# vainglorygame/analyzer

Measured on AMD Instinct MI355X. Metric: matches/sec rated (whole node), 3v3 TrueSkill, 1M-player roster, higher is better.
Workload: dtype fp32; 1 GPU; global_batch=10000000, seq_len=6, players=1000000, matches_per_gpu=10000000, team_size=3, parallelism=dp1, mode=exact, bench_config=2, skew=1, force_merge=False

## Files before the change

### analyzer_amd/csrc/dataflow.hip

```cpp
#include <hip/hip_runtime.h>

#include "common.h"
#include "dataflow_dev.h"
#include "kernels.h"
#include "rate_core.h"
#include "rate_dev.h"
#include "telemetry_dev.h"

#ifndef ANA_HELD
#define ANA_HELD 1
#endif

namespace ana {

#ifndef ANA_LOCAL_HANDOFF
#define ANA_LOCAL_HANDOFF 1
#endif
constexpr bool kLocalHandoff = ANA_LOCAL_HANDOFF != 0;
#ifndef ANA_LOCAL_HANDOFF_MAXK
#define ANA_LOCAL_HANDOFF_MAXK 4
#endif


constexpr int kHeld = ANA_HELD;
#ifndef ANA_HELD5
#define ANA_HELD5 1
#endif
constexpr int kTeleInline = 64;

struct Batch {
  int32_t m = 0;
  int my_h = -1, my_bit = 0, mode = 0, n0 = 0, n1 = 0, rank0 = 1, rank1 = 1, first = 0, prevdup = -1;
  int32_t id = -1;
  bool inr = false, islast = false, own = false, any_dup = false;
  uint32_t lk0 = kNoMatch;
  v4i gs = {0, 0, 0, 0}, gm = {0, 0, 0, 0};
  int64_t toff = 0;
  int32_t tcnt = 0;
  bool tonly = false;
  uint8_t est = kRated;
};

template <int K, int G, int TELE, bool DIAG, int WPE = 1>
__global__ void __launch_bounds__(256) __attribute__((amdgpu_waves_per_eu(WPE)))
rate_dataflow_kernel(const int32_t* __restrict__ rec, const uint32_t* __restrict__ link,
                     int32_t* deps, float* state, const float* __restrict__ attrs,
                     float* __restrict__ first_prior, float* __restrict__ orows, int64_t orow,
                     uint32_t* ctrl,
                     RateParams prm, TelemetryParams tp) {
  constexpr int S = 2 * K;
  constexpr int R = S + 2;
  constexpr int kH = K >= 5 ? ANA_HELD5 : kHeld;
  constexpr bool kLH = kLocalHandoff && (K <= ANA_LOCAL_HANDOFF_MAXK || ANA_DIAG_BUILD != 0);
  constexpr bool TILES = TELE == 1;
  constexpr bool INL = TELE == 2;
  static_assert(G >= S && G <= 64, "a group holds one match");
  constexpr int NG = 64 / G;
  static_assert(kH >= 1 && kH <= 4, "held chunks");
  typedef uint32_t hvec __attribute__((ext_vector_type(kH <= 2 ? 2 : 4)));
  __shared__ hvec lloc[kWavesPerBlock][kLH ? kChunk : 1];
  constexpr int SPT = (4 + S + 3) / 4 * 4;
  constexpr int SP = SPT + (INL ? 4 : 0);
  constexpr int TT = INL ? ((kTeleInline + G - 1) / G < 8 ? (kTeleInline + G - 1) / G : 8) : 1;
  __shared__ __attribute__((aligned(16))) float tstat[kWavesPerBlock][INL ? NG : 1][INL ? S * kStatFeatures : 4];
  __shared__ __attribute__((aligned(16))) int32_t lpick[kWavesPerBlock][NG][SP];
  __shared__ float tele[kWavesPerBlock][TILES ? tele_scratch_floats<K>() : 1];
  constexpr int OQ = (5 * S + 2 + 3) / 4;
  __shared__ __attribute__((aligned(16))) float lrow[kWavesPerBlock][NG][4 * OQ];
  const int lane = threadIdx.x & 63;
  const int wv = threadIdx.x >> 6;
  const int j = lane % G;
  const int g = lane / G;
  const int gbase = lane - j;
  const uint64_t gmask = (((1ull << G) - 1ull) << gbase);
  const bool r0 = j < K;
  const int rpos = r0 ? j : j - K;
  const int64_t M = prm.num_matches;
  const int64_t P = prm.num_players;
  const float beta2 = prm.beta2, tau2 = prm.tau2, us = prm.unknown_sigma;
  const int epoch = prm.epoch_ptr ? __builtin_amdgcn_readfirstlane(*prm.epoch_ptr) : prm.epoch;
  const __amdgpu_buffer_rsrc_t rs =
      __builtin_amdgcn_make_buffer_rsrc(state, 0, (int)(P * kRowFloats * 4), 0x00020000);
  const __amdgpu_buffer_rsrc_t rl = __builtin_amdgcn_make_buffer_rsrc(
      const_cast<uint32_t*>(link), 0, (int)(M * S * 4), 0x00020000);
  const __amdgpu_buffer_rsrc_t rd = __builtin_amdgcn_make_buffer_rsrc(deps, 0, (int)(M * 4), 0x00020000);
  const int head = blockIdx.x % kHeads;
  uint64_t t0 = __builtin_amdgcn_s_memrealtime();
  uint32_t seen_progress = 0;
  const bool local_ok = kLH && prm.local_handoff != 0;
  uint32_t n_local = 0, n_global = 0, n_stale = 0;
  uint64_t d_issue = 0, d_wait = 0, d_after = 0, d_it0 = 0;
  uint64_t d_t[4] = {0, 0, 0, 0}, d_p[5] = {0, 0, 0, 0, 0};
  uint64_t d_s[4] = {0, 0, 0, 0}, d_i[3] = {0, 0, 0};
  uint32_t d_worked = 0, d_groups = 0, d_near = 0, d_pend = 0;

  int32_t hrec[kH][R];
  int64_t hoff[kH];
  int32_t hcnt[kH];
  int32_t cbase[kH];
  uint64_t pend[kH];
  uint32_t dval[kH];
  uint32_t need[kH];
#pragma unroll
  for (int h = 0; h < kH; ++h) {
    cbase[h] = -1;
    pend[h] = 0ull;
#pragma unroll
    for (int k = 0; k < R; ++k) hrec[h][k] = -1;
    dval[h] = kNone;
    need[h] = 0u;
    hoff[h] = 0;
    hcnt[h] = 0;
  }
  bool exhausted = false, tk_pending = false;
  unsigned tk = 0;
  uint32_t spins = 0, iter = 0;
  const bool tele_role = TILES && tp.role_stride > 0 && tp.impl != 0;
  const bool tele_inline = INL && tp.role_stride < 0 && tp.evoff != nullptr;
  const int tele_span = tele_role ? kTeleMaxSpan : kTeleTile;
  const int64_t tele_tiles = TILES && tp.evoff ? (tp.num_matches + tele_span - 1) / tele_span : 0;
  bool tele_done = tele_tiles == 0 || tele_inline;
  auto tele_claim = [&]() -> int64_t {
    unsigned t = 0;
    if (lane == 0)
      t = __hip_atomic_fetch_add((gu32*)&ctrl[12], 1u, __ATOMIC_RELAXED, __HIP_MEMORY_SCOPE_AGENT);
    t = __builtin_amdgcn_readfirstlane(t);
    return (int64_t)t < tele_tiles ? (int64_t)t : -1;
  };
  auto tele_run = [&](int64_t t) {
    if constexpr (TILES) {
      if (tele_role) telemetry_tile_mfma<K, 0, kTeleMaxSpan>(tp, t, lane, tele[wv], &ctrl[13]);
      else if (tp.impl) telemetry_tile_mfma<K>(tp, t, lane, tele[wv], &ctrl[13]);
      else telemetry_tile<K>(tp, t, lane, tele[wv], &ctrl[13]);
    }
  };
  if constexpr (TILES) {
    if (tele_role) {
      const int b = blockIdx.x, per = tp.role_stride >= 4 ? tp.role_stride / 4 : 1;
      const bool agg = tp.role_stride >= 4   ? (wv == ((b >> 3) & 3) && ((b >> 5) % per) == 0)
                       : tp.role_stride == 2 ? ((wv & 1) == ((b >> 3) & 1))
                                             : true;
      while (agg && !tele_done) {
        const int64_t t = tele_claim();
        if (t < 0) tele_done = true;
        else tele_run(t);
      }
    }
  }
  v2u tev_prev[TT];
#pragma unroll
  for (int t = 0; t < TT; ++t) tev_prev[t] = v2u{0u, 0u};
  int32_t tp_m = -1, tp_cnt = 0;
  int64_t tp_off = 0;
  auto tele_flush = [&]() {
    if constexpr (INL) {
      if (tp_m < 0) return;
      float* const ts = tstat[wv][g];
      typedef float v4f __attribute__((ext_vector_type(4)));
      if (j < S) {
        reinterpret_cast<v4f*>(ts)[2 * j] = v4f{0.f, 0.f, 0.f, 0.f};
        reinterpret_cast<v4f*>(ts)[2 * j + 1] = v4f{0.f, 0.f, 0.f, 0.f};
      }
      uint32_t nbad = 0;
      const uint32_t mtag = (uint32_t)tp_m & 0xffffu;
      auto fold = [&](v2u ev) {
        const int32_t meta = (int32_t)ev.x;
        const int slot = event_slot(meta);
        if (event_tag(meta) != mtag || slot >= S) {
          ++nbad;
          return;
        }
        float add;
        const int f = event_feature(event_type(meta), __uint_as_float(ev.y), add);
        if (f >= 0) atomicAdd(&ts[slot * kStatFeatures + f], add);
        atomicAdd(&ts[slot * kStatFeatures + kStatEvents], 1.f);
      };
#pragma unroll
      for (int t = 0; t < TT; ++t)
        if (j + G * t < tp_cnt) fold(tev_prev[t]);
      for (int e = j + G * TT; e < tp_cnt; e += G)
        fold(__builtin_nontemporal_load(reinterpret_cast<const v2u*>(tp.events + 2 * (tp_off + e))));
      if (j < S) {
        v4f* dst = reinterpret_cast<v4f*>(tp.stats + ((int64_t)tp_m * S + j) * kStatFeatures);
        __builtin_nontemporal_store(reinterpret_cast<const v4f*>(ts)[2 * j], dst);
        __builtin_nontemporal_store(reinterpret_cast<const v4f*>(ts)[2 * j + 1], dst + 1);
      }
      if (nbad) atomicAdd(&ctrl[13], nbad);
      tp_m = -1;
    }
  };
  const uint32_t max_spins = prm.idle_spins > 0 ? (uint32_t)prm.idle_spins : 0u;
  const int cl = prm.chunk_len;
  const int64_t nchunks = (M + cl - 1) / cl;

  for (;;) {
    if constexpr (DIAG) d_it0 = __builtin_amdgcn_s_memrealtime();
    uint64_t ready[kH];
    {
      hvec lv = {};
      if constexpr (kLH) lv = lloc[wv][lane];
#pragma unroll
      for (int h = 0; h < kH; ++h)
        ready[h] = __ballot(dval[h] != kNone && dval[h] + lv[h] == need[h]) & pend[h];
      if constexpr (DIAG) {
        uint32_t nn = 0, np = 0;
#pragma unroll
        for (int h = 0; h < kH; ++h) {
          nn += (uint32_t)__popcll(__ballot(dval[h] != kNone && dval[h] + lv[h] + 1u == need[h]) & pend[h]);
          np += (uint32_t)__popcll(pend[h]);
        }
        bool any = false;
#pragma unroll
        for (int h = 0; h < kH; ++h) any |= ready[h] != 0ull;
        if (any) {
          d_near += nn;
          d_pend += np;
        }
      }
    }
    __builtin_amdgcn_fence(__ATOMIC_ACQUIRE, "wavefront");
    if constexpr (DIAG) d_i[0] = __builtin_amdgcn_s_memrealtime();

    int my_h = -1, my_bit = 0, nassigned = 0;
#pragma unroll
    for (int h = 0; h < kH; ++h) {
      const uint64_t rdy = ready[h];
      if (rdy != 0ull && nassigned < NG) {
        const uint32_t below = __builtin_amdgcn_mbcnt_hi(
            (uint32_t)(rdy >> 32), __builtin_amdgcn_mbcnt_lo((uint32_t)rdy, 0u));
        const bool mine = ((rdy >> lane) & 1ull) && nassigned + (int)below < NG;
        if (mine) {
          int32_t w[SP];
          w[0] = cbase[h] + lane;
          w[1] = (h << 8) | lane;
          w[2] = hrec[h][S];
          w[3] = hrec[h][S + 1];
#pragma unroll
          for (int k = 0; k < SPT - 4; ++k) w[4 + k] = k < S ? hrec[h][k] : -1;
          if constexpr (INL) {
            w[SPT] = (int32_t)(uint32_t)hoff[h];
            w[SPT + 1] = (int32_t)(hoff[h] >> 32);
            w[SPT + 2] = hcnt[h];
            w[SPT + 3] = 0;
          }
          v4i* dst = reinterpret_cast<v4i*>(&lpick[wv][nassigned + (int)below][0]);
#pragma unroll
          for (int q = 0; q < SP / 4; ++q) dst[q] = v4i{w[4 * q], w[4 * q + 1], w[4 * q + 2], w[4 * q + 3]};
        }
        const uint64_t taken = __ballot(mine);
        pend[h] &= ~taken;
        nassigned += __popcll(taken);
      }
    }
    int32_t my_m = 0, my_id = -1;
    uint32_t my_m0 = 0u, my_m1 = 0u;
    int64_t my_toff = 0;
    int32_t my_tcnt = 0;
    if (g < nassigned) {
      const v4i pk = *reinterpret_cast<const v4i*>(&lpick[wv][g][0]);
      if constexpr (INL) {
        const v4i tk4 = *reinterpret_cast<const v4i*>(&lpick[wv][g][SPT]);
        my_toff = (int64_t)(((uint64_t)(uint32_t)tk4.y << 32) | (uint32_t)tk4.x);
        my_tcnt = tk4.z;
      }
      if (j < S) my_id = lpick[wv][g][4 + j];
      my_m = pk.x;
      my_h = (pk.y >> 8) & 255;
      my_bit = pk.y & 255;
      my_m0 = (uint32_t)pk.z;
      my_m1 = (uint32_t)pk.w;
    }
    const bool worked = nassigned > 0;
    if constexpr (DIAG) {
      d_worked += worked ? 1u : 0u;
      d_groups += (uint32_t)nassigned;
      d_i[1] = __builtin_amdgcn_s_memrealtime();
    }

    Batch nb;
    {
      const int32_t m = my_m;
      const uint32_t m0 = my_m0, m1 = my_m1;
      const int mode = meta_mode(m0);
      nb.my_h = my_h;
      nb.my_bit = my_bit;
      nb.m = m;
      nb.mode = mode;
      nb.n0 = meta_n0(m0);
      nb.n1 = meta_n1(m0);
      nb.rank0 = meta_winner0(m1) ? 0 : 1;
      nb.rank1 = meta_winner1(m1) ? 0 : 1;
      nb.tonly = INL && ((m1 >> 4) & 1u);
      nb.est = (uint8_t)(m1 >> 28);
      nb.tcnt = my_h >= 0 ? my_tcnt : 0;
      nb.toff = my_toff;
      const bool inr = my_h >= 0 && j < S && rpos < (r0 ? nb.n0 : nb.n1) && !nb.tonly;
      nb.inr = inr;
      const int32_t id = inr ? my_id : -1;
      nb.id = id;
      bool islast = true;
      int first = j, prevdup = -1;
      nb.any_dup = __ballot((m1 >> 3) & 1u) != 0ull;
      if (nb.any_dup) {
#pragma unroll
        for (int q = 0; q < S; ++q) {
          const int32_t oid = __shfl(id, gbase + q);
          if (id >= 0 && oid == id) {
            if (q < j) {
              if (first == j) first = q;
              prevdup = q;
            }
            if (q > j) islast = false;
          }
        }
      }
      nb.islast = islast;
      nb.first = first;
      nb.prevdup = prevdup;
      const bool own = inr && first == j;
      nb.own = own;
      const int goff = own ? id * (kRowFloats * 4) : kOutOfRange;
      nb.gs = __builtin_amdgcn_raw_buffer_load_b128(rs, goff, 0, 16);
      nb.gm = __builtin_amdgcn_raw_buffer_load_b128(rs, goff + 16 * (1 + mode), 0, 16);
      nb.lk0 = __builtin_amdgcn_raw_buffer_load_b32(rl, inr ? (m * S + j) * 4 : kOutOfRange, 0, 0);
    }

    if constexpr (DIAG) d_i[2] = __builtin_amdgcn_s_memrealtime();
    int staging = -1;
    int32_t r[R];
    uint32_t lks[S];
    int64_t stoff = 0;
    int32_t stcnt = 0;
#pragma unroll
    for (int k = 0; k < R; ++k) r[k] = -1;
#pragma unroll
    for (int k = 0; k < S; ++k) lks[k] = 0u;
    if (tk_pending) {
      const unsigned t = __builtin_amdgcn_readfirstlane(tk);
      tk_pending = false;
      const int64_t c = (int64_t)t * kHeads + head;
      if (prm.progress && lane == 0 &&
          ((c >= prm.progress_at && c < prm.progress_at + kHeads) ||
           (c >= nchunks && c < nchunks + kHeads)))
        __hip_atomic_store(prm.progress, prm.progress_value, __ATOMIC_RELAXED,
                           __HIP_MEMORY_SCOPE_SYSTEM);
      if (c * cl >= M) {
        exhausted = true;
      } else {
#pragma unroll
        for (int h = kH - 1; h >= 0; --h)
          if (cbase[h] < 0) staging = h;
#pragma unroll
        for (int h = 0; h < kH; ++h)
          if (h == staging) cbase[h] = (int32_t)(c * cl);
        const int64_t m = c * cl + lane;
        if (lane < cl && m < M) {
          const int32_t* src = rec + m * R;
          if constexpr (R % 4 == 0) {
#pragma unroll
            for (int k = 0; k < R / 4; ++k) {
              const v4i v = reinterpret_cast<const v4i*>(src)[k];
              r[4 * k] = v.x; r[4 * k + 1] = v.y; r[4 * k + 2] = v.z; r[4 * k + 3] = v.w;
            }
          } else {
#pragma unroll
            for (int k = 0; k < R; ++k) r[k] = src[k];
          }
          const v2u* ls = reinterpret_cast<const v2u*>(link + m * S);
#pragma unroll
          for (int k = 0; k < S / 2; ++k) {
            const v2u v = ls[k];
            lks[2 * k] = v.x;
            lks[2 * k + 1] = v.y;
          }
          if (tele_inline) {
            stoff = tp.evoff[m];
            stcnt = (int32_t)(tp.evoff[m + 1] - stoff);
          }
        }
      }
    }

    v2u tev_next[TT];
    int32_t tn_m = -1, tn_cnt = 0;
    int64_t tn_off = 0;
    auto notify = [&](uint32_t succ) {
      if (succ == kNoMatch) return;
      int lh = -1;
      int32_t lcb = 0;
      if (kLH && local_ok) {
#pragma unroll
        for (int h = 0; h < kH; ++h)
          if (cbase[h] >= 0 && (int32_t)succ >= cbase[h] && (int32_t)succ < cbase[h] + cl) {
            lh = h;
            lcb = cbase[h];
          }
      }
      if (kLH && lh >= 0) {
        atomicAdd(reinterpret_cast<uint32_t*>(&lloc[wv][(int32_t)succ - lcb]) + lh, 1u);
      } else {
        __hip_atomic_fetch_add((gu32*)(deps + succ), 1u, __ATOMIC_RELAXED, __HIP_MEMORY_SCOPE_AGENT);
      }
      const uint64_t lb = __ballot(lh >= 0);
      n_local += (uint32_t)__popcll(lb);
      n_global += (uint32_t)__popcll(__ballot(true) & ~lb);
    };
    auto rate_batch = [&](const Batch& bt) {
    int my_h = bt.my_h;
    const int my_bit = bt.my_bit;
    const int32_t m = bt.m;
    const int mode = bt.mode, n0 = bt.n0, n1 = bt.n1, rank0 = bt.rank0, rank1 = bt.rank1;
    const int first = bt.first, prevdup = bt.prevdup;
    const int32_t id = bt.id;
    const bool inr = bt.inr, islast = bt.islast, own = bt.own, any_dup = bt.any_dup;
    const uint32_t lk0 = bt.lk0;
    const v4i gs = bt.gs, gm = bt.gm;
    const uint32_t sa = (uint32_t)gs.y;
    const bool s_this = (sa & 0xffu) == (uint32_t)epoch;
    const uint32_t counters = s_this ? sa >> 8 : 0u;
    const uint32_t cnt = (counters >> (4 * mode)) & 15u;
    const bool shared_ok = !(lk0 & kLinkHasPred) || (s_this && (uint32_t)gs.w == (uint32_t)m);
    const bool mode_ok = cnt == 0u || (gm.y == epoch && (uint32_t)gm.w == cnt);
    const bool fresh = !own || (shared_ok && mode_ok);
    const bool overtaken =
        own && (((lk0 & kLinkHasPred) && s_this && (uint32_t)gs.w != kNoMatch &&
                 (uint32_t)gs.w > (uint32_t)m) ||
                (shared_ok && gm.y == epoch && (uint32_t)gm.w == (cnt == 15u ? 1u : cnt + 1u)));
    if (__ballot(overtaken) != 0ull && lane == 0) {
      atomicOr(&ctrl[2], 1u);
      atomicOr(&ctrl[18], 1u);
    }
    const uint64_t stale_lanes = __ballot(!fresh);
    if (stale_lanes) {
      const bool gstale = (stale_lanes & gmask) != 0ull;
      n_stale += (uint32_t)__popcll(__ballot(gstale && j == 0));
#pragma unroll
      for (int h = 0; h < kH; ++h) {
        uint64_t back = 0ull;
        for (int q = 0; q < NG; ++q) {
          const int bq = __shfl(gstale && my_h == h ? my_bit : -1, q * G);
          if (bq >= 0) back |= 1ull << bq;
        }
        pend[h] |= uniform64(back);
      }
      if (gstale) my_h = -1;
    }
    if constexpr (INL) {
      if (tele_inline && my_h >= 0) {
        tn_m = m;
        tn_cnt = bt.tcnt;
        tn_off = bt.toff;
      }
#pragma unroll
      for (int t = 0; t < TT; ++t) {
        const bool okl = tele_inline && my_h >= 0 && j + G * t < bt.tcnt;
        const int32_t* src = okl ? tp.events + 2 * (bt.toff + j + G * t)
                                 : reinterpret_cast<const int32_t*>(tp.evoff);
        tev_next[t] = __builtin_nontemporal_load(reinterpret_cast<const v2u*>(src));
      }
    }
    if (my_h >= 0) {
      const float smu = __int_as_float(gs.x), ssg = __int_as_float(gs.z);
      const float mmu = __int_as_float(gm.x), msg = __int_as_float(gm.z);
      const bool sh_null = smu != smu, md_null = mmu != mmu;
      float pms = smu, pss = ssg;
      bool seed_ok = true;
      if (__ballot(own && sh_null) != 0ull && own && sh_null) {
        const float4 at4 = reinterpret_cast<const float4*>(attrs)[id];
        const float attr[4] = {at4.x, at4.y, at4.z, at4.w};
        seed_ok = seed_prior<float>(attr, us, prm.vst, pms, pss);
      }
      const bool sh_bad = !sh_null && !(ssg == ssg && ssg != 0.f);
      const bool md_bad = !md_null && !(msg == msg && msg != 0.f);
      float pmm = md_null ? pms : mmu, psm = md_null ? pss : msg;
      uint32_t pflags = own ? ((sh_null ? 2u : 1u) | (md_null ? 4u : 0u)) : 0u;
      const uint8_t lst = !own ? (uint8_t)kRated
                               : (sh_null && !seed_ok) ? (uint8_t)kErrSeed
                               : (sh_bad || md_bad) ? (uint8_t)kErrSigma : (uint8_t)kRated;
      const uint64_t eb = __ballot(lst != kRated) & gmask;
      uint8_t gst = kRated;
      if (eb) gst = (uint8_t)__shfl((int)lst, (int)__builtin_ctzll(eb));
      float rsmu = smu, rssg = ssg, rmmu = mmu, rmsg = msg;
      uint32_t rcnt = counters;
      if (any_dup) {
        const int src = gbase + first;
        pms = __shfl(pms, src);
        pss = __shfl(pss, src);
        pmm = __shfl(pmm, src);
        psm = __shfl(psm, src);
        pflags = (uint32_t)__shfl((int)pflags, src);
        rsmu = __shfl(smu, src);
        rssg = __shfl(ssg, src);
        rcnt = (uint32_t)__shfl((int)counters, src);
        rmmu = __shfl(mmu, src);
        rmsg = __shfl(msg, src);
      }
      if (bt.tonly) gst = bt.est;
      if (gst == kRated && (n0 == 0 || n1 == 0)) gst = kErrEmptyRoster;
      float nsm = NAN, nss = NAN, nmm = NAN, nms = NAN, dl = NAN, q = NAN;
      if (gst == kRated) {
        if constexpr (DIAG) d_p[1] = __builtin_amdgcn_s_memrealtime();
        const float lsg = (r0 == (rank0 <= rank1)) ? 1.f : -1.f;
        f2 nm2, ns2;
        rate_pair<G>(f2{pms, pmm}, f2{pss, psm}, inr, lsg, n0 + n1, rank0 == rank1, beta2, tau2, j,
                     gbase, nm2, ns2, q);
        nsm = nm2.x;
        nmm = nm2.y;
        nss = ns2.x;
        nms = ns2.y;
        const bool bad_num = inr && !(isfinite(nsm) && isfinite(nss) && isfinite(nmm) &&
                                      isfinite(nms) && isfinite(q));
        if ((__ballot(bad_num) & gmask) != 0ull) gst = kErrNumeric;
        const float cur = nsm - nss;
        const float prevw = any_dup ? __shfl(cur, gbase + (prevdup >= 0 ? prevdup : j)) : cur;
        if (prevdup >= 0) dl = cur - prevw;
        else if (pflags & 1u) dl = cur - (pms - pss);
        else dl = 0.f;
      }
      const bool ok = gst == kRated && inr;
      if constexpr (DIAG) d_p[2] = __builtin_amdgcn_s_memrealtime();
      if (inr && islast) {
        const int off = id * (kRowFloats * 4);
        const uint32_t succ = lk0 & kMatchMask;
        const uint32_t c4 = (rcnt >> (4 * mode)) & 15u;
        const uint32_t c = c4 == 15u ? 1u : c4 + 1u;
        const uint32_t ncnt = (rcnt & ~(15u << (4 * mode))) | (c << (4 * mode));
        const uint32_t stag = (uint32_t)epoch | (ncnt << 8);
        __builtin_amdgcn_raw_buffer_store_b128(
            ok ? granule(nmm, (uint32_t)epoch, nms, c) : granule(rmmu, (uint32_t)epoch, rmsg, c),
            rs, off + 16 * (1 + mode), 0, 16);
        __builtin_amdgcn_raw_buffer_store_b128(
            ok ? granule(nsm, stag, nss, succ) : granule(rsmu, stag, rssg, succ),
            rs, off, 0, 16);
        notify(lk0 & kMatchMask);
      }
      if constexpr (DIAG) d_p[3] = __builtin_amdgcn_s_memrealtime();
      if (ok && prm.record_first_prior && own) {
        float* fp = first_prior + (int64_t)id * kRowFloats;
        if (pflags & 2u) { fp[0] = pms; fp[2] = pss; }
        if (pflags & 4u) { fp[4 * (1 + mode)] = pmm; fp[4 * (1 + mode) + 2] = psm; }
      }
      float* const orm = orows + (int64_t)m * orow;
      float* const lr = lrow[wv][g];
      if (j < S) {
        lr[j] = ok ? nsm : NAN;
        lr[S + j] = ok ? nss : NAN;
        lr[2 * S + j] = ok ? dl : NAN;
        lr[3 * S + j] = ok ? nmm : NAN;
        lr[4 * S + j] = ok ? nms : NAN;
      }
      if (j == 0) {
        lr[5 * S] = gst == kRated ? q : (gst == kAfk || gst == kInvalidRosters) ? 0.f : NAN;
        lr[5 * S + 1] = __uint_as_float((uint32_t)gst);
      }
      if (j == (G > 1 ? 1 : 0)) {
#pragma unroll
        for (int k = 5 * S + 2; k < 4 * OQ; ++k) lr[k] = 0.f;
      }
#pragma unroll
      for (int t = 0; t < (OQ + G - 1) / G; ++t) {
        typedef float v4f __attribute__((ext_vector_type(4)));
        const int qd = j + t * G;
        if (qd < OQ)
          __builtin_nontemporal_store(reinterpret_cast<const v4f*>(lr)[qd], reinterpret_cast<v4f*>(orm) + qd);
      }
    }
    };

    {
      bool free_slot = false;
#pragma unroll
      for (int h = 0; h < kH; ++h) free_slot |= cbase[h] < 0;
      if (free_slot && !exhausted) {
        if (lane == 0)
          tk = __hip_atomic_fetch_add((gu32*)&ctrl[4 + head], 1u, __ATOMIC_RELAXED,
                                      __HIP_MEMORY_SCOPE_AGENT);
        tk_pending = true;
      }
    }

    uint64_t d_w0 = 0, d_w1 = 0;
    if constexpr (DIAG) d_w0 = __builtin_amdgcn_s_memrealtime();
    asm volatile("s_waitcnt vmcnt(0)" ::: "memory");
    if constexpr (DIAG) d_w1 = __builtin_amdgcn_s_memrealtime();
    if constexpr (INL) {
#pragma unroll
      for (int t = 0; t < TT; ++t) asm volatile("" : "+v"(tev_prev[t]));
    }

    int64_t early_m = -1;
    uint8_t early_est = kRated;
    if (staging >= 0) {
      int64_t cb = 0;
#pragma unroll
      for (int h = 0; h < kH; ++h) if (h == staging) cb = cbase[h];
      const int64_t mm = lane < cl ? cb + lane : M;
      uint32_t nd = 0u;
      {
        const uint32_t m0s = (uint32_t)r[S];
        bool dup = false;
#pragma unroll
        for (int a = 0; a < S; ++a) {
          const bool ina = (a < K ? a : a - K) < (a < K ? meta_n0(m0s) : meta_n1(m0s));
          bool firsto = ina;
#pragma unroll
          for (int b = 0; b < a; ++b) {
            const bool inb = (b < K ? b : b - K) < (b < K ? meta_n0(m0s) : meta_n1(m0s));
            dup |= r[a] >= 0 && r[a] == r[b];
            if (inb && r[b] == r[a]) firsto = false;
          }
          if (firsto && (lks[a] & kLinkHasPred)) ++nd;
        }
        r[S + 1] = dup ? (r[S + 1] | 8) : (r[S + 1] & ~8);
      }
      const uint8_t est = mm < M ? early_status<K>(r, P) : kRated;
      const bool tonly = tele_inline && mm < M && est != kRated;
      if (tonly) r[S + 1] = (int32_t)(((uint32_t)r[S + 1] & 0x0fffffffu) | 16u | ((uint32_t)est << 28));
#pragma unroll
      for (int h = 0; h < kH; ++h)
        if (h == staging) {
#pragma unroll
          for (int k = 0; k < R; ++k) hrec[h][k] = r[k];
          hoff[h] = stoff;
          hcnt[h] = stcnt;
        }
      if constexpr (kLH) reinterpret_cast<uint32_t*>(&lloc[wv][lane])[staging] = 0u;
      if (mm < M && est != kRated && !tonly) {
        early_m = mm;
        early_est = est;
      }
      const uint64_t pm = __ballot(mm < M && (est == kRated || tonly));
#pragma unroll
      for (int h = 0; h < kH; ++h)
        if (h == staging) {
          pend[h] = pm;
          dval[h] = kNone;
          need[h] = tonly ? 0u : nd;
          if (pm == 0ull) cbase[h] = -1;
        }
    }

    if constexpr (DIAG) d_p[0] = d_p[1] = d_p[2] = d_p[3] = d_w1;
    rate_batch(nb);
    if (early_m >= 0) {
      typedef float v4f __attribute__((ext_vector_type(4)));
      const float qv = (early_est == kAfk || early_est == kInvalidRosters) ? 0.f : NAN;
      v4f* dst = reinterpret_cast<v4f*>(orows + early_m * orow);
#pragma unroll
      for (int q = 0; q < OQ; ++q) {
        float v[4];
#pragma unroll
        for (int i = 0; i < 4; ++i) {
          const int pos = 4 * q + i;
          v[i] = pos < 5 * S ? NAN : pos == 5 * S ? qv : pos == 5 * S + 1 ? __uint_as_float((uint32_t)early_est) : 0.f;
        }
        __builtin_nontemporal_store(v4f{v[0], v[1], v[2], v[3]}, dst + q);
      }
    }
    if constexpr (INL) {
      tele_flush();
#pragma unroll
      for (int t = 0; t < TT; ++t) tev_prev[t] = tev_next[t];
      tp_m = tn_m;
      tp_cnt = tn_cnt;
      tp_off = tn_off;
    }
    if constexpr (DIAG) {
      if (worked) {
        const uint64_t end = __builtin_amdgcn_s_memrealtime();
        d_issue += d_w0 - d_it0;
        d_wait += d_w1 - d_w0;
        d_after += end - d_w1;
        d_s[0] += d_i[0] - d_it0;
        d_s[1] += d_i[1] - d_i[0];
        d_s[2] += d_i[2] - d_i[1];
        d_s[3] += d_w0 - d_i[2];
        const uint64_t p1 = __builtin_amdgcn_readfirstlane((uint32_t)d_p[1]) |
                            ((uint64_t)__builtin_amdgcn_readfirstlane((uint32_t)(d_p[1] >> 32)) << 32);
        const uint64_t p2 = __builtin_amdgcn_readfirstlane((uint32_t)d_p[2]) |
                            ((uint64_t)__builtin_amdgcn_readfirstlane((uint32_t)(d_p[2] >> 32)) << 32);
        const uint64_t p3 = __builtin_amdgcn_readfirstlane((uint32_t)d_p[3]) |
                            ((uint64_t)__builtin_amdgcn_readfirstlane((uint32_t)(d_p[3] >> 32)) << 32);
        if (p1 >= d_w1 && p2 >= p1 && p3 >= p2 && end >= p3) {
          d_t[0] += p1 - d_w1;
          d_t[1] += p2 - p1;
          d_t[2] += p3 - p2;
          d_t[3] += end - p3;
        }
      }
    }

    ++iter;
#pragma unroll
    for (int h = 0; h < kH; ++h)
      dval[h] = __builtin_amdgcn_raw_buffer_load_b32(rd, ((pend[h] >> lane) & 1ull) ? (cbase[h] + lane) * 4 : kOutOfRange,
                                                     0, 16);

    {
      uint32_t retired = 0;
#pragma unroll
      for (int h = 0; h < kH; ++h)
        if (cbase[h] >= 0 && pend[h] == 0ull) {
          cbase[h] = -1;
          ++retired;
        }
      retired = __builtin_amdgcn_readfirstlane(retired);
      if (retired && lane == 0)
        __hip_atomic_fetch_add((gu32*)&ctrl[3], retired, __ATOMIC_RELAXED, __HIP_MEMORY_SCOPE_AGENT);
    }

    bool held = false;
#pragma unroll
    for (int h = 0; h < kH; ++h) held |= cbase[h] >= 0;
    if (exhausted && !held && !tk_pending) {
      tele_flush();
      if (lane == 0) {
        __hip_atomic_fetch_add((gu32*)&ctrl[15], iter, __ATOMIC_RELAXED, __HIP_MEMORY_SCOPE_AGENT);
        __hip_atomic_fetch_add((gu32*)&ctrl[26], n_local, __ATOMIC_RELAXED, __HIP_MEMORY_SCOPE_AGENT);
        __hip_atomic_fetch_add((gu32*)&ctrl[27], n_global, __ATOMIC_RELAXED, __HIP_MEMORY_SCOPE_AGENT);
        if (n_stale) __hip_atomic_fetch_add((gu32*)&ctrl[14], n_stale, __ATOMIC_RELAXED, __HIP_MEMORY_SCOPE_AGENT);
        if constexpr (DIAG) {
          __hip_atomic_fetch_add((gu32*)&ctrl[20], d_worked, __ATOMIC_RELAXED, __HIP_MEMORY_SCOPE_AGENT);
          __hip_atomic_fetch_add((gu32*)&ctrl[21], d_groups, __ATOMIC_RELAXED, __HIP_MEMORY_SCOPE_AGENT);
          __hip_atomic_fetch_add((gu32*)&ctrl[30], d_near, __ATOMIC_RELAXED, __HIP_MEMORY_SCOPE_AGENT);
          __hip_atomic_fetch_add((gu32*)&ctrl[31], d_pend, __ATOMIC_RELAXED, __HIP_MEMORY_SCOPE_AGENT);
          atomicAdd(reinterpret_cast<unsigned long long*>(&ctrl[22]), (unsigned long long)d_issue);
          atomicAdd(reinterpret_cast<unsigned long long*>(&ctrl[24]), (unsigned long long)d_wait);
          atomicAdd(reinterpret_cast<unsigned long long*>(&ctrl[28]), (unsigned long long)d_after);
          for (int q = 0; q < 4; ++q)
            atomicAdd(reinterpret_cast<unsigned long long*>(&ctrl[32 + 2 * q]), (unsigned long long)d_t[q]);
          for (int q = 0; q < 4; ++q)
            atomicAdd(reinterpret_cast<unsigned long long*>(&ctrl[40 + 2 * q]), (unsigned long long)d_s[q]);
        }
      }
      if constexpr (TILES) {
        while (!tele_done) {
          const int64_t t = tele_claim();
          if (t < 0) tele_done = true;
          else tele_run(t);
        }
      }
      break;
    }

    if (worked || staging >= 0) {
      spins = 0;
    } else {
      const uint64_t now = __builtin_amdgcn_s_memrealtime();
      if (now - t0 > kProgressTicks) {
        const uint32_t p = __hip_atomic_load((gu32*)&ctrl[3], __ATOMIC_RELAXED, __HIP_MEMORY_SCOPE_AGENT);
        if (p != seen_progress) {
          seen_progress = p;
          t0 = now;
        }
      }
      if (now - t0 > kTimeoutTicks) {
        if (lane == 0) {
          atomicOr(&ctrl[1], 1u);
          atomicOr(&ctrl[17], 1u);
        }
#pragma unroll
        for (int h = 0; h < kH; ++h)
          if (cbase[h] >= 0 && ((pend[h] >> lane) & 1ull))
            reinterpret_cast<uint8_t*>(orows + (int64_t)(cbase[h] + lane) * orow + 5 * S + 1)[0] = kNotProcessed;
        return;
      }
      if constexpr (TILES) {
        if (!tele_done && ((!tp.fused_tail && !tele_role) || !held)) {
          const int64_t t = tele_claim();
          if (t >= 0) {
            tele_run(t);
            spins = 0;
            continue;
          }
          tele_done = true;
        }
      }
      spins = spins < max_spins ? spins + 1u : max_spins;
      for (uint32_t k = 0; k < spins; ++k) __builtin_amdgcn_s_sleep(2);
    }
  }
}


__global__ void __launch_bounds__(64) zero_ctrl2_kernel(uint32_t* __restrict__ a, int na,
                                                        uint32_t* __restrict__ b, int nb) {
  if ((int)threadIdx.x < na) a[threadIdx.x] = 0u;
  if ((int)threadIdx.x < nb) b[threadIdx.x] = 0u;
}

int launch_rate(int K, const int32_t* rec, const uint32_t* link, int32_t* deps, float* state,
                const float* attrs, float* first_prior, const RateOut& out, uint32_t* ctrl,
                const RateParams& prm, const TelemetryParams& tp, int blocks, hipStream_t s) {
  const int64_t M = prm.num_matches;
  hipLaunchKernelGGL(zero_ctrl2_kernel, dim3(1), dim3(64), 0, s, ctrl + 1, prm.ctrl_ready ? 0 : 15,
                     ctrl + 20, 32);
  if (M <= 0) return 0;
  if (prm.chunk_len < 1 || prm.chunk_len > kChunk) return (int)hipErrorInvalidValue;
  if ((int64_t)prm.num_players * kRowFloats * 4 > kOutOfRange) return (int)hipErrorInvalidValue;
  if (M * 2 * K * 4 > kOutOfRange) return (int)hipErrorInvalidValue;
  if (!prm.epoch_ptr && (prm.epoch < 1 || prm.epoch > 255)) return (int)hipErrorInvalidValue;
  const int S = 2 * K;
  if (!(out.s_sig == out.s_mu + S && out.delta == out.s_mu + 2 * S && out.m_mu == out.s_mu + 3 * S &&
        out.m_sig == out.s_mu + 4 * S && out.quality == out.s_mu + 5 * S && out.qrow == out.row &&
        (void*)out.status == (void*)(out.s_mu + 5 * S + 1) && out.srow == out.row * 4))
    return (int)hipErrorInvalidValue;
  if (blocks < kHeads) blocks = kHeads;
  const bool tight = prm.tight_groups > 0 || (prm.tight_groups < 0 && K == 5);
#define ANA_RATE_LAUNCH_W(k, g, tele, diag, w)                                                     \
  hipLaunchKernelGGL((rate_dataflow_kernel<k, g, tele, diag, w>), dim3((unsigned)blocks), dim3(256), 0, s, \
                     rec, link, deps, state, attrs, first_prior, out.s_mu, out.row, ctrl, prm, tp)
#define ANA_RATE_LAUNCH_D(k, g, tele, diag)                                                        \
  do {                                                                                             \
    if constexpr (tele == 0 && !diag && k <= 3 && (g & (g - 1)) == 0) {                            \
      if (blocks > 256) ANA_RATE_LAUNCH_W(k, g, tele, diag, 4);           \
      else ANA_RATE_LAUNCH_W(k, g, tele, diag, 1);                                                 \
    } else {                                                                                       \
      ANA_RATE_LAUNCH_W(k, g, tele, diag, 1);                                                      \
    }                                                                                              \
  } while (0)
#define ANA_RATE_LAUNCH(k, g)                                      \
  do {                                                             \
    if (tp.evoff && tp.role_stride < 0) ANA_RATE_LAUNCH_D(k, g, 2, false); \
    else if (tp.evoff) ANA_RATE_LAUNCH_D(k, g, 1, false);          \
    else if (prm.diag) ANA_RATE_LAUNCH_D(k, g, 0, true);           \
    else ANA_RATE_LAUNCH_D(k, g, 0, false);                        \
  } while (0)
  switch (K) {
    case 1: ANA_RATE_LAUNCH(1, 2); break;
    case 2: ANA_RATE_LAUNCH(2, 4); break;
    case 3:
      if (tight) ANA_RATE_LAUNCH(3, 6);
      else ANA_RATE_LAUNCH(3, 8);
      break;
    case 4: ANA_RATE_LAUNCH(4, 8); break;
    case 5:
      if (tight) ANA_RATE_LAUNCH(5, 10);
      else ANA_RATE_LAUNCH(5, 16);
      break;
    default: return (int)hipErrorInvalidValue;
  }
#undef ANA_RATE_LAUNCH
#undef ANA_RATE_LAUNCH_D
  return (int)hipGetLastError();
}

}
```

### analyzer_amd/ops/rate.py

```python
from __future__ import annotations

import os
from dataclasses import dataclass
from typing import Dict, NamedTuple, Optional, Tuple

import torch

from ..config import MODES, N_TRACKS, EngineConfig, RaterConfig
from ..models.tiers import vst_table
from .native import native

RATED, AFK, INVALID_ROSTERS, UNSUPPORTED_MODE = 0, 1, 2, 3
ERR_SEED, ERR_SIGMA, ERR_EMPTY_ROSTER, ERR_NUMERIC, ERR_BAD_RECORD = 4, 5, 6, 7, 8
NOT_PROCESSED = 255
CTRL_WORDS = 52
STATUS_NAMES = {RATED: "rated", AFK: "afk", INVALID_ROSTERS: "invalid_rosters",
                UNSUPPORTED_MODE: "unsupported_mode", ERR_SEED: "error_seed",
                ERR_SIGMA: "error_sigma", ERR_EMPTY_ROSTER: "error_empty_roster",
                ERR_NUMERIC: "error_numeric", ERR_BAD_RECORD: "error_bad_record",
                NOT_PROCESSED: "not_processed"}
ERROR_STATUSES = (ERR_SEED, ERR_SIGMA, ERR_EMPTY_ROSTER, ERR_NUMERIC, ERR_BAD_RECORD)


class NativeRateError(RuntimeError):
    pass


class Schedule(NamedTuple):
    link: torch.Tensor
    deps: torch.Tensor

    NO_MATCH = 0x0FFFFFFF
    MATCH_MASK = 0x0FFFFFFF
    HAS_PRED = 1 << 30


@dataclass
class Roster:

    state: torch.Tensor
    attrs: torch.Tensor
    epoch: Optional[int] = None

    ROW = 32

    @property
    def num_players(self) -> int:
        return int(self.state.shape[0])

    @property
    def device(self) -> torch.device:
        return self.state.device

    @staticmethod
    def empty(num_players: int, device="cpu") -> "Roster":
        state = torch.zeros((num_players, 32), dtype=torch.float32, device=device)
        state[:, 0::2] = float("nan")
        attrs = torch.full((num_players, 4), float("nan"), dtype=torch.float32, device=device)
        attrs[:, 3] = 0.0
        return Roster(state, attrs, epoch=0)

    def tracks(self) -> torch.Tensor:
        return self.state.view(-1, 8, 4)[:, :, 0::2]

    def mu(self) -> torch.Tensor:
        return self.state[:, 0::4]

    def sigma(self) -> torch.Tensor:
        return self.state[:, 2::4]

    def track(self, name: str) -> torch.Tensor:
        idx = 0 if name in ("shared", "trueskill") else 1 + MODES.index(name.replace("trueskill_", ""))
        return self.state[:, 4 * idx:4 * idx + 3:2]

    def to(self, device) -> "Roster":
        return Roster(self.state.to(device), self.attrs.to(device), self.epoch)

    def clone(self) -> "Roster":
        return Roster(self.state.clone(), self.attrs.clone(), self.epoch)

    def next_epoch(self) -> int:
        if self.epoch is None or self.epoch >= 255:
            native().reset_tags(self.state)
            self.epoch = 0
        self.epoch += 1
        return self.epoch


@dataclass
class RateResult:

    quality: torch.Tensor
    status: torch.Tensor
    s_mu: torch.Tensor
    s_sig: torch.Tensor
    delta: torch.Tensor
    m_mu: torch.Tensor
    m_sig: torch.Tensor
    packed: Optional[torch.Tensor] = None

    FIELDS = ("quality", "status", "s_mu", "s_sig", "delta", "m_mu", "m_sig")

    @staticmethod
    def row_floats(K: int) -> int:
        return -(-(5 * 2 * K + 2) // 32) * 32

    @staticmethod
    def allocate(M: int, K: int, device, packed: bool = True) -> "RateResult":
        S = 2 * K
        if not packed:
            f = dict(dtype=torch.float32, device=device)
            return RateResult(torch.empty(M, **f), torch.empty(M, dtype=torch.uint8, device=device),
                              *(torch.empty((M, S), **f) for _ in range(5)))
        W = RateResult.row_floats(K)
        return RateResult.from_packed(torch.empty((M, W), dtype=torch.float32, device=device), K)

    @staticmethod
    def from_packed(buf: torch.Tensor, K: int) -> "RateResult":
        S = 2 * K
        if buf.dim() != 2 or buf.shape[1] != RateResult.row_floats(K) or buf.dtype != torch.float32 \
                or not buf.is_contiguous():
            raise ValueError("packed rows must be a contiguous fp32 [M, %d]" % RateResult.row_floats(K))
        slots = [buf[:, f * S:(f + 1) * S] for f in range(5)]
        status = buf.view(torch.uint8)[:, 4 * (5 * S + 1)]
        return RateResult(buf[:, 5 * S], status, *slots, packed=buf)

    @property
    def any_afk(self) -> torch.Tensor:
        return (self.status == AFK) | (self.status == INVALID_ROSTERS)

    def status_counts(self) -> Dict[str, int]:
        vals, counts = torch.unique(self.status.cpu(), return_counts=True)
        return {STATUS_NAMES.get(int(v), str(int(v))): int(c) for v, c in zip(vals, counts)}


class BatchRater:

    def __init__(self, cfg: Optional[RaterConfig] = None, host_fp64: bool = True,
                 blocks: Optional[int] = None):
        self.cfg = cfg or RaterConfig.from_env()
        self.host_fp64 = host_fp64
        ecfg = EngineConfig.from_env()
        self.fixed_blocks = int(blocks or ecfg.rate_blocks or 0)
        self.blocks = self.fixed_blocks or 512
        self.knobs = ecfg.rate_knobs()
        self.tele_fuse_max = int(ecfg.tele_fuse_max)
        self.chunk_cap = int(os.environ.get("ANA_RATE_CHUNK") or 0)
        self._vst: Dict[str, torch.Tensor] = {}
        self._ws: Dict[Tuple[str, str], torch.Tensor] = {}

    @staticmethod
    def has_telemetry(telemetry) -> bool:
        return telemetry is not None and telemetry[0].numel() > 0

    def tiles(self, telemetry, M: int) -> bool:
        return self.has_telemetry(telemetry) and self.knobs[5] >= 0

    def fuses(self, telemetry, M: int) -> bool:
        return self.has_telemetry(telemetry) and (self.knobs[5] >= 0 or M <= self.tele_fuse_max)

    def launch_blocks(self, K: int = 3, roster_bytes: int = 0) -> int:
        if self.fixed_blocks:
            return self.fixed_blocks
        return 256 if roster_bytes <= (256 << 20) else 512

    def chunk_len(self, M: int, telemetry: bool = False, blocks: Optional[int] = None, K: int = 3) -> int:
        if telemetry:
            return 64
        cap = self.chunk_cap if self.chunk_cap > 0 else (32 if K >= 5 else 64)
        need = -(-M // (4 * (blocks or self.blocks)))
        cl = 8
        while cl < need and cl < 64:
            cl *= 2
        return max(8, min(cl, cap))

    def grid_blocks(self, M: int, telemetry: bool = False, blocks: Optional[int] = None, K: int = 3) -> int:
        if telemetry:
            return self.blocks
        b = blocks or self.blocks
        chunks = -(-M // self.chunk_len(M, blocks=b, K=K))
        return max(1, min(b, -(-chunks // 4)))

    def vst(self, device) -> torch.Tensor:
        key = str(device)
        if key not in self._vst:
            self._vst[key] = torch.tensor(vst_table(), dtype=torch.float32, device=device)
        return self._vst[key]

    def _buffer(self, device, name: str, numel: int, dtype) -> torch.Tensor:
        key = (str(device), name)
        buf = self._ws.get(key)
        if buf is None or buf.numel() < numel or buf.dtype != dtype:
            buf = torch.empty(int(numel), dtype=dtype, device=device)
            self._ws[key] = buf
        return buf[:numel]

    def _ctrl(self, device) -> torch.Tensor:
        key = (str(device), "ctrl")
        buf = self._ws.get(key)
        if buf is None:
            buf = torch.zeros(CTRL_WORDS, dtype=torch.int32, device=device)
            self._ws[key] = buf
        return buf

    def schedule(self, rec: torch.Tensor, K: int, num_players: int,
                 tag: str = "", zero_ctrl: bool = False,
                 epoch_bump: Optional[torch.Tensor] = None, sort_nt: int = -1) -> Schedule:
        M = rec.shape[0]
        dev = rec.device
        link = self._buffer(dev, "link" + tag, M * 2 * K, torch.int32).view(M, 2 * K)
        deps = self._buffer(dev, "deps" + tag, M, torch.int32)
        if rec.is_cuda:
            nbytes = native().schedule_workspace_bytes(M * 2 * K, num_players)
            ws = self._buffer(dev, "sched_ws", nbytes, torch.uint8)
            ctrl = self._ctrl(dev)
        else:
            ws = torch.empty(0, dtype=torch.uint8)
            ctrl = torch.empty(0, dtype=torch.int32)
        bump = epoch_bump.data_ptr() if epoch_bump is not None and rec.is_cuda else 0
        native().schedule(rec, K, num_players, link, deps, ws, ctrl, bool(zero_ctrl and rec.is_cuda),
                          bump, int(sort_nt))
        return Schedule(link, deps)

    def rate(self, roster: Roster, rec: torch.Tensor, K: Optional[int] = None,
             out: Optional[RateResult] = None, first_prior: Optional[torch.Tensor] = None,
             check: bool = True, schedule: Optional[Schedule] = None,
             telemetry=None, progress=None, epoch_dev: Optional[torch.Tensor] = None) -> RateResult:
        K = int(K or (rec.shape[1] - 2) // 2)
        M = int(rec.shape[0])
        dev = rec.device
        if roster.device != dev:
            raise ValueError("roster is on %s but the stream is on %s" % (roster.device, dev))
        if out is None:
            out = RateResult.allocate(M, K, dev)
        P = roster.num_players
        cfg = self.cfg
        record = first_prior is not None
        fp = first_prior if record else torch.empty(0, dtype=torch.float32, device=dev)
        if dev.type == "cuda":
            ctrl_ready = schedule is None
            if schedule is None:
                schedule = self.schedule(rec, K, P, zero_ctrl=True, epoch_bump=epoch_dev)
            elif epoch_dev is not None:
                native().epoch_bump(epoch_dev)
            link, deps = schedule
            ctrl = self._ctrl(dev)
            epoch = roster.next_epoch() if epoch_dev is None else 1
        else:
            link = deps = ctrl = torch.empty(0, dtype=torch.int32)
            epoch = 1
            ctrl_ready = False
        blocks = self.launch_blocks(K, roster.state.numel() * roster.state.element_size())
        tiles = self.tiles(telemetry, M)
        after = None
        if self.has_telemetry(telemetry) and not self.fuses(telemetry, M) and dev.type == "cuda":
            after, telemetry = telemetry, None
        tele = self.has_telemetry(telemetry)
        if not tele:
            none = torch.empty(0, dtype=torch.int64, device=dev)
            telemetry = (none, none.to(torch.int32), none.to(torch.float32))
        native().rate(rec, K, link, deps, roster.state, roster.attrs, fp, out.quality, out.status,
                      out.s_mu, out.s_sig, out.delta, out.m_mu, out.m_sig, ctrl, self.vst(dev),
                      float(cfg.beta) ** 2, float(cfg.tau) ** 2, float(cfg.unknown_player_sigma),
                      record, self.grid_blocks(M, tiles, blocks, K), epoch,
                      self.host_fp64, *telemetry,
                      *(progress if progress is not None and dev.type == "cuda" else (0, 0, 0)),
                      epoch_dev.data_ptr() if epoch_dev is not None and dev.type == "cuda" else 0,
                      self.chunk_len(M, tiles, blocks, K), ctrl_ready, self.knobs)
        if after is not None:
            evoff, events, stats = after
            native().telemetry(evoff, events, K, stats, ctrl[13:14])
        if check and dev.type == "cuda":
            self.check_errors(dev)
        return out

    def stale_retries(self, device) -> int:
        return int(self._ctrl(device)[14].item())

    def iterations(self, device) -> int:
        return int(self._ctrl(device)[15].item())

    def handoffs(self, device) -> Tuple[int, int]:
        c = self._ctrl(device)[26:28].cpu()
        return int(c[0]), int(c[1])

    def diag(self, device) -> Dict[str, float]:
        c = [int(x) & 0xffffffff for x in self._ctrl(device).cpu().tolist()]
        u64 = lambda i: c[i] | (c[i + 1] << 32)
        worked = c[20]
        per = (lambda t: t * 0.01 / worked) if worked else (lambda t: 0.0)
        return {"wave_iterations": c[15], "worked_iterations": worked, "groups_assigned": c[21],
                "matches_per_worked_iteration": c[21] / worked if worked else 0.0,
                "issue_us": per(u64(22)), "wait_us": per(u64(24)), "after_us": per(u64(28)),
                "after_prior_us": per(u64(32)), "after_update_us": per(u64(34)),
                "after_publish_us": per(u64(36)), "after_rest_us": per(u64(38)),
                "issue_ready_us": per(u64(40)), "issue_assign_us": per(u64(42)),
                "issue_loads_us": per(u64(44)), "issue_polls_us": per(u64(46)),
                "local_handoffs": c[26], "global_handoffs": c[27],
                "near_ready_per_worked_iteration": c[30] / worked if worked else 0.0,
                "pending_per_worked_iteration": c[31] / worked if worked else 0.0,
                "stale_retries": c[14]}

    def telemetry_errors(self, device) -> int:
        return int(self._ctrl(device)[13].item())

    def error_flags(self, device) -> torch.Tensor:
        return self._ctrl(device)[0:3]

    def sticky_flags(self, device) -> torch.Tensor:
        return self._ctrl(device)[16:19]

    def clear_sticky(self, device) -> None:
        self._ctrl(device)[16:19].zero_()

    def check_errors(self, device, sticky: bool = False) -> None:
        self.raise_flags((self.sticky_flags(device) if sticky else self.error_flags(device)).cpu())

    @staticmethod
    def raise_flags(flags: torch.Tensor) -> None:
        if int(flags[0]):
            raise NativeRateError("schedule prepass failed (flag %d)" % int(flags[0]))
        if int(flags[1]):
            raise NativeRateError("dataflow rating timed out (a dependency never resolved)")
        if int(flags[2]):
            raise NativeRateError("dataflow race detected: a player's granule was written by a "
                                  "later match before an earlier one read it")


def rate_stream(roster: Roster, rec: torch.Tensor, K: Optional[int] = None,
                cfg: Optional[RaterConfig] = None) -> RateResult:
    return BatchRater(cfg).rate(roster, rec, K)


__all__ = ["Roster", "RateResult", "BatchRater", "rate_stream", "STATUS_NAMES", "N_TRACKS"]
```

Before: 1.598 billion matches/s.

## Add fast path for plain full-roster fresh batches in dataflow rater

Adds a compile-time fast path in the rate_batch lambda, enabled by default for non-telemetry, non-diag builds. When every active lane in the wave has a full, fresh, valid, non-duplicated 3v3 roster, it calls rate_pair, writes the state granules, notifies successors, stores the output row and returns early. This skips the general stale-handling, prior, telemetry and error-status logic. It also replaces short-circuit boolean logic with bitwise ops to cut branches, returns early when the wave did no work, and counts fast-path batches in a new ctrl word. The risk is extra code size and register pressure, plus a possible behaviour mismatch with the general path in edge cases.

```diff
diff --git a/analyzer_amd/csrc/dataflow.hip b/analyzer_amd/csrc/dataflow.hip
--- a/analyzer_amd/csrc/dataflow.hip
+++ b/analyzer_amd/csrc/dataflow.hip
@@ -21,6 +21,9 @@
 #define ANA_LOCAL_HANDOFF_MAXK 4
 #endif
 
+#ifndef ANA_PLAIN_FAST
+#define ANA_PLAIN_FAST 1
+#endif
 
 constexpr int kHeld = ANA_HELD;
 #ifndef ANA_HELD5
@@ -52,6 +55,7 @@
   constexpr int R = S + 2;
   constexpr int kH = K >= 5 ? ANA_HELD5 : kHeld;
   constexpr bool kLH = kLocalHandoff && (K <= ANA_LOCAL_HANDOFF_MAXK || ANA_DIAG_BUILD != 0);
+  constexpr bool kFast = ANA_PLAIN_FAST != 0 && ANA_DIAG_BUILD == 0 && TELE == 0 && !DIAG && WPE == 1;
   constexpr bool TILES = TELE == 1;
   constexpr bool INL = TELE == 2;
   static_assert(G >= S && G <= 64, "a group holds one match");
@@ -89,6 +93,7 @@
   uint32_t seen_progress = 0;
   const bool local_ok = kLH && prm.local_handoff != 0;
   uint32_t n_local = 0, n_global = 0, n_stale = 0;
+  uint32_t n_plain = 0;
   uint64_t d_issue = 0, d_wait = 0, d_after = 0, d_it0 = 0;
   uint64_t d_t[4] = {0, 0, 0, 0}, d_p[5] = {0, 0, 0, 0, 0};
   uint64_t d_s[4] = {0, 0, 0, 0}, d_i[3] = {0, 0, 0};
@@ -406,6 +411,9 @@
       n_global += (uint32_t)__popcll(__ballot(true) & ~lb);
     };
     auto rate_batch = [&](const Batch& bt) {
+    if constexpr (kFast) {
+      if (!worked) return;
+    }
     int my_h = bt.my_h;
     const int my_bit = bt.my_bit;
     const int32_t m = bt.m;
@@ -419,16 +427,85 @@
     const bool s_this = (sa & 0xffu) == (uint32_t)epoch;
     const uint32_t counters = s_this ? sa >> 8 : 0u;
     const uint32_t cnt = (counters >> (4 * mode)) & 15u;
-    const bool shared_ok = !(lk0 & kLinkHasPred) || (s_this && (uint32_t)gs.w == (uint32_t)m);
-    const bool mode_ok = cnt == 0u || (gm.y == epoch && (uint32_t)gm.w == cnt);
-    const bool fresh = !own || (shared_ok && mode_ok);
-    const bool overtaken =
-        own && (((lk0 & kLinkHasPred) && s_this && (uint32_t)gs.w != kNoMatch &&
-                 (uint32_t)gs.w > (uint32_t)m) ||
-                (shared_ok && gm.y == epoch && (uint32_t)gm.w == (cnt == 15u ? 1u : cnt + 1u)));
+    const bool has_pred = (lk0 & kLinkHasPred) != 0u;
+    const bool m_this = gm.y == epoch;
+    bool shared_ok, mode_ok, fresh, overtaken;
+    if constexpr (DIAG) {
+      shared_ok = !has_pred || (s_this && (uint32_t)gs.w == (uint32_t)m);
+      mode_ok = cnt == 0u || (m_this && (uint32_t)gm.w == cnt);
+      fresh = !own || (shared_ok && mode_ok);
+      overtaken = own && ((has_pred && s_this && (uint32_t)gs.w != kNoMatch && (uint32_t)gs.w > (uint32_t)m) ||
+                          (shared_ok && m_this && (uint32_t)gm.w == (cnt == 15u ? 1u : cnt + 1u)));
+    } else {
+      shared_ok = !has_pred | (s_this & ((uint32_t)gs.w == (uint32_t)m));
+      mode_ok = (cnt == 0u) | (m_this & ((uint32_t)gm.w == cnt));
+      fresh = !own | (shared_ok & mode_ok);
+      overtaken =
+          own & ((has_pred & s_this & ((uint32_t)gs.w != kNoMatch) & ((uint32_t)gs.w > (uint32_t)m)) |
+                 (shared_ok & m_this & ((uint32_t)gm.w == (cnt == 15u ? 1u : cnt + 1u))));
+    }
     if (__ballot(overtaken) != 0ull && lane == 0) {
       atomicOr(&ctrl[2], 1u);
       atomicOr(&ctrl[18], 1u);
+    }
+    if constexpr (kFast) {
+      const bool act = my_h >= 0 && j < S;
+      const float smu = __int_as_float(gs.x), ssg = __int_as_float(gs.z);
+      const float mmu = __int_as_float(gm.x), msg = __int_as_float(gm.z);
+      const bool valid = (smu == smu) & (mmu == mmu) & (ssg == ssg) & (ssg != 0.f) & (msg == msg) & (msg != 0.f);
+      const bool lane_plain = (n0 == K) & (n1 == K) & fresh & !overtaken & valid;
+      if (!any_dup && __ballot(act & !lane_plain) == 0ull) {
+        const float lsg = (r0 == (rank0 <= rank1)) ? 1.f : -1.f;
+        f2 nm2, ns2;
+        float q;
+        rate_pair<G>(f2{smu, mmu}, f2{ssg, msg}, act, lsg, n0 + n1, rank0 == rank1, beta2, tau2, j,
+                     gbase, nm2, ns2, q);
+        const float nsm = nm2.x, nmm = nm2.y, nss = ns2.x, nms = ns2.y;
+        const bool bad_num = act && !(isfinite(nsm) && isfinite(nss) && isfinite(nmm) &&
+                                      isfinite(nms) && isfinite(q));
+        if (__ballot(bad_num) == 0ull) {
+          ++n_plain;
+          if (act) {
+            const int off = id * (kRowFloats * 4);
+            const uint32_t succ = lk0 & kMatchMask;
+            const uint32_t c = cnt == 15u ? 1u : cnt + 1u;
+            const uint32_t ncnt = (counters & ~(15u << (4 * mode))) | (c << (4 * mode));
+            const uint32_t stag = (uint32_t)epoch | (ncnt << 8);
+            __builtin_amdgcn_raw_buffer_store_b128(granule(nmm, (uint32_t)epoch, nms, c), rs,
+                                                   off + 16 * (1 + mode), 0, 16);
+            __builtin_amdgcn_raw_buffer_store_b128(granule(nsm, stag, nss, succ), rs, off, 0, 16);
+            notify(succ);
+          }
+          if (my_h >= 0) {
+            float* const orm = orows + (int64_t)m * orow;
+            float* const lr = lrow[wv][g];
+            if (j < S) {
+              const float cur = nsm - nss;
+              lr[j] = nsm;
+              lr[S + j] = nss;
+              lr[2 * S + j] = cur - (smu - ssg);
+              lr[3 * S + j] = nmm;
+              lr[4 * S + j] = nms;
+            }
+            if (j == 0) {
+              lr[5 * S] = q;
+              lr[5 * S + 1] = __uint_as_float((uint32_t)kRated);
+            }
+            if (j == (G > 1 ? 1 : 0)) {
+#pragma unroll
+              for (int k = 5 * S + 2; k < 4 * OQ; ++k) lr[k] = 0.f;
+            }
+#pragma unroll
+            for (int t = 0; t < (OQ + G - 1) / G; ++t) {
+              typedef float v4f __attribute__((ext_vector_type(4)));
+              const int qd = j + t * G;
+              if (qd < OQ)
+                __builtin_nontemporal_store(reinterpret_cast<const v4f*>(lr)[qd], reinterpret_cast<v4f*>(orm) + qd);
+            }
+          }
+          return;
+        }
+      }
     }
     const uint64_t stale_lanes = __ballot(!fresh);
     if (stale_lanes) {
@@ -719,6 +796,7 @@
         __hip_atomic_fetch_add((gu32*)&ctrl[26], n_local, __ATOMIC_RELAXED, __HIP_MEMORY_SCOPE_AGENT);
         __hip_atomic_fetch_add((gu32*)&ctrl[27], n_global, __ATOMIC_RELAXED, __HIP_MEMORY_SCOPE_AGENT);
         if (n_stale) __hip_atomic_fetch_add((gu32*)&ctrl[14], n_stale, __ATOMIC_RELAXED, __HIP_MEMORY_SCOPE_AGENT);
+        if (n_plain) __hip_atomic_fetch_add((gu32*)&ctrl[48], n_plain, __ATOMIC_RELAXED, __HIP_MEMORY_SCOPE_AGENT);
         if constexpr (DIAG) {
           __hip_atomic_fetch_add((gu32*)&ctrl[20], d_worked, __ATOMIC_RELAXED, __HIP_MEMORY_SCOPE_AGENT);
           __hip_atomic_fetch_add((gu32*)&ctrl[21], d_groups, __ATOMIC_RELAXED, __HIP_MEMORY_SCOPE_AGENT);
diff --git a/analyzer_amd/ops/rate.py b/analyzer_amd/ops/rate.py
--- a/analyzer_amd/ops/rate.py
+++ b/analyzer_amd/ops/rate.py
@@ -277,6 +277,9 @@
     def stale_retries(self, device) -> int:
         return int(self._ctrl(device)[14].item())
 
+    def plain_batches(self, device) -> int:
+        return int(self._ctrl(device)[48].item())
+
     def iterations(self, device) -> int:
         return int(self._ctrl(device)[15].item())
 
```

After: 1.611 billion matches/s, median of 6. No clear change (+0.8%).
